# scroll-tech/zkevm-circuits

Hardware: AMD Instinct MI355X
Metric: SuperCircuit-shape proof-gen wall-clock (s) at k = 20 (lower is better)
Workload: dtype u32x8 limbs (254-bit modular integer, Montgomery)

## Files before the change

zkevm-circuits_amd/csrc/ntt.hip:

```cpp
#include "ctx.hpp"
#include "ff29.hip.hpp"

namespace zk {

constexpr int NTT_MAX_DIGIT = 10;
constexpr int NTT_TILE = 4096;
constexpr int NTT_THREADS = 1024;
constexpr int NTT_LDS_BYTES_PER_ELT = 36;

struct Tw29;

constexpr int NTT_BATCH = 16;
struct NttIo { const Fr* src[NTT_BATCH]; Fr* dst[NTT_BATCH]; };

struct NttPass {
    int log_np;
    int log_m;
    const Tw29* tw;
    const Fr* out_tw = nullptr;
};

struct NttDomain {
    uint32_t log_n = 0;
    int npass = 0;
    NttPass pass[3];
    int h = 0;
    Fr* d_lo = nullptr;
    Fr* d_hi = nullptr;
    Fr* d_tw[3] = {nullptr, nullptr, nullptr};
    Tw29* d_tw29[3] = {nullptr, nullptr, nullptr};
    Fr* d_out_tw[2] = {nullptr, nullptr};
    Fr final_mul;
    bool fin_folded = false;
    ~NttDomain() {
        if (d_lo) (void)hipFree(d_lo);
        if (d_hi) (void)hipFree(d_hi);
        for (auto p : d_tw) if (p) (void)hipFree(p);
        for (auto p : d_tw29) if (p) (void)hipFree((void*)p);
        for (auto p : d_out_tw) if (p) (void)hipFree(p);
    }
};

__device__ __forceinline__ uint32_t bitrev(uint32_t x, int bits) { return bits ? (__brev(x) >> (32 - bits)) : 0u; }

__host__ __device__ __forceinline__ Fr to_rprime(Fr x) {
#pragma unroll
    for (int i = 0; i < 5; ++i) x = dbl(x);
    return x;
}

struct Lds29 {
    uint32_t* p;
    int stride;
    __device__ __forceinline__ Fr29 load(int idx) const {
        Fr29 r;
#pragma unroll
        for (int k = 0; k < 9; ++k) r.l[k] = p[k * stride + idx];
        return r;
    }
    __device__ __forceinline__ void store(int idx, const Fr29& v) const {
#pragma unroll
        for (int k = 0; k < 9; ++k) p[k * stride + idx] = v.l[k];
    }
};

__global__ void k_powers(Fr base, Fr mul, Fr* out, uint32_t count, int rprime) {
    uint32_t j = blockIdx.x * blockDim.x + threadIdx.x;
    if (j >= count) return;
    Fr r = mul, b = base;
    uint32_t e = j;
    while (e) {
        if (e & 1) r = r * b;
        b = sqr(b);
        e >>= 1;
    }
    stg(out + j, rprime ? to_rprime(r) : r);
}

__device__ __forceinline__ Fr two_level(const Fr* __restrict__ lo, const Fr* __restrict__ hi, int h, uint32_t e) {
    return ldg(lo + (e & ((1u << h) - 1))) * ldg(hi + (e >> h));
}
__device__ __forceinline__ Fr29 two_level29(const Fr* __restrict__ lo, const Fr* __restrict__ hi, int h, uint32_t e) {
    return mul29(unpack29<Fr29P>(ldg(lo + (e & ((1u << h) - 1)))), unpack29<Fr29P>(ldg(hi + (e >> h))));
}

__global__ void k_build_out_twiddles(Fr* __restrict__ out_tw, const Fr* __restrict__ lo, const Fr* __restrict__ hi, int h, int log_np, int log_m, int tw_shift, uint64_t n,
                                     Fr fin, int apply_fin) {
    const uint64_t g = (uint64_t)blockIdx.x * blockDim.x + threadIdx.x;
    if (g >= n) return;
    const uint64_t m = 1ull << log_m;
    const uint32_t jpp = (uint32_t)(g & (m - 1)), d = (uint32_t)(g >> log_m) & ((1u << log_np) - 1);
    Fr29 v = two_level29(lo, hi, h, (jpp * d) << tw_shift);
    if (apply_fin) v = mul29(v, unpack29<Fr29P>(fin));
    stg(out_tw + g, pack29_lt2p(v));
}

__device__ __forceinline__ void bfly29(Fr29& u, Fr29& x, const Fr29& w) {
    const Fr29 v = mul29(x, w);
    Fr29 a0 = add29(u, v), a1 = sub29k<4>(u, v);
    normalize29(a0);
    normalize29(a1);
    u = a0;
    x = a1;
}
struct Tw29 { uint4 q[3]; };
__device__ __forceinline__ Fr29 tw29(const Tw29* __restrict__ tw, uint32_t idx) {
    const uint4 a = tw[idx].q[0], b = tw[idx].q[1], c = tw[idx].q[2];
    return Fr29{{a.x, a.y, a.z, a.w, b.x, b.y, b.z, b.w, c.x}};
}
__global__ void k_split_twiddles(const Fr* __restrict__ in, Tw29* __restrict__ out, uint32_t count) {
    const uint32_t i = blockIdx.x * blockDim.x + threadIdx.x;
    if (i >= count) return;
    const Fr29 v = unpack29<Fr29P>(ldg(in + i));
    out[i].q[0] = make_uint4(v.l[0], v.l[1], v.l[2], v.l[3]);
    out[i].q[1] = make_uint4(v.l[4], v.l[5], v.l[6], v.l[7]);
    out[i].q[2] = make_uint4(v.l[8], 0u, 0u, 0u);
}
__device__ __forceinline__ void bfly29_lazy(Fr29& u, Fr29& x, const Fr29& w) {
    const Fr29 v = mul29(x, w);
    const Fr29 a0 = add29(u, v), a1 = sub29k<2>(u, v);
    u = a0;
    x = a1;
}
template <int R>
__device__ __forceinline__ void dit_step(Fr29 (&e)[4], const Tw29* __restrict__ tw, int log_np, int s, int j) {
    const Fr29 w0 = tw29(tw, (uint32_t)j << (log_np - 1 - s));
    bfly29_lazy(e[0], e[1], w0);
    if (R == 2) {
        bfly29_lazy(e[2], e[3], w0);
        bfly29_lazy(e[0], e[2], tw29(tw, (uint32_t)j << (log_np - 2 - s)));
        bfly29_lazy(e[1], e[3], tw29(tw, (uint32_t)(j + (1 << s)) << (log_np - 2 - s)));
        normalize29(e[2]);
        normalize29(e[3]);
    }
    normalize29(e[0]);
    normalize29(e[1]);
}
__device__ __forceinline__ void bfly29_one(Fr29& u, Fr29& x) {
    Fr29 a0 = add29(u, x), a1 = sub29k<4>(u, x);
    normalize29(a0);
    normalize29(a1);
    u = a0;
    x = a1;
}
template <int R>
__device__ __forceinline__ void dit_first_step(Fr29 (&e)[4], const Tw29* __restrict__ tw, int log_np) {
    bfly29_one(e[0], e[1]);
    if (R == 2) {
        bfly29_one(e[2], e[3]);
        bfly29_one(e[0], e[2]);
        bfly29(e[1], e[3], tw29(tw, 1u << (log_np - 2)));
    }
}

__global__ void __launch_bounds__(NTT_THREADS)
k_ntt_pass(NttIo io, const Tw29* __restrict__ tw, const Fr* __restrict__ lo,
           const Fr* __restrict__ hi, int h, int log_np, int log_t, int log_m, int tw_shift, const Fr* __restrict__ pre,
           const Fr* __restrict__ out_tw, uint32_t ncols, int xcd_cols) {
    extern __shared__ __attribute__((aligned(16))) uint32_t smem[];
    uint32_t tile_id, col;
    if (xcd_cols) { const uint32_t slot = blockIdx.x >> 3; col = slot % ncols; tile_id = (slot / ncols) * 8u + (blockIdx.x & 7u); }
    else { col = blockIdx.x % ncols; tile_id = blockIdx.x / ncols; }
    const Fr* __restrict__ src = io.src[col];
    Fr* __restrict__ dst = io.dst[col];
    const int tile = 1 << (log_np + log_t);
    Lds29 L{smem, tile};
    const int T = 1 << log_t;
    const uint64_t m = 1ull << log_m;
    const uint32_t tiles_per_hi = (uint32_t)(m >> log_t);
    const uint32_t hi_idx = tile_id / tiles_per_hi, blk = tile_id % tiles_per_hi;
    const uint64_t base = ((uint64_t)hi_idx << (log_np + log_m)) + ((uint64_t)blk << log_t);

    for (int s = 0; s < log_np;) {
        const int r = ((log_np - s) & 1) ? 1 : 2;
        const bool first = s == 0, last = s + r == log_np;
        const int hgt = 1 << s, items = tile >> r;
        for (int it = threadIdx.x; it < items; it += blockDim.x) {
            const int c = it & (T - 1), b = it >> log_t;
            const int j = b & (hgt - 1);
            const int lo_d = ((b >> s) << (s + r)) | j;
            Fr29 e[4];
#pragma unroll
            for (int k = 0; k < 4; ++k) {
                if (k >= (1 << r)) break;
                const int dl = lo_d + k * hgt;
                if (first) {
                    const uint64_t gi = base + (uint64_t)bitrev(dl, log_np) * m + c;
                    e[k] = unpack29<Fr29P>(ldg(src + gi));
                    if (pre) e[k] = mul29(e[k], unpack29<Fr29P>(ldg(pre + gi)));
                } else {
                    e[k] = L.load((dl << log_t) | c);
                }
            }
            if (first) { if (r == 2) dit_first_step<2>(e, tw, log_np); else dit_first_step<1>(e, tw, log_np); }
            else if (r == 2) dit_step<2>(e, tw, log_np, s, j);
            else dit_step<1>(e, tw, log_np, s, j);
#pragma unroll
            for (int k = 0; k < 4; ++k) {
                if (k >= (1 << r)) break;
                const int dl = lo_d + k * hgt;
                if (last) {
                    const uint32_t jpp = (blk << log_t) + c;
                    const uint64_t go = base + (uint64_t)dl * m + c;
                    const Fr29 v = mul29(e[k], out_tw ? unpack29<Fr29P>(ldg(out_tw + go)) : two_level29(lo, hi, h, (jpp * (uint32_t)dl) << tw_shift));
                    stg(dst + go, pack29_raw(v));
                } else {
                    L.store((dl << log_t) | c, e[k]);
                }
            }
        }
        s += r;
        if (s < log_np) __syncthreads();
    }
}

static bool ntt_xcd_remap() { static const bool on = getenv("ZK_NTT_XCD") && atoi(getenv("ZK_NTT_XCD")) == 1; return on; }
__host__ __device__ __forceinline__ int ntt_row_pad(int log_np) { return log_np >= 8 ? 8 : 0; }
__global__ void __launch_bounds__(NTT_THREADS)
k_ntt_last(NttIo io, const Tw29* __restrict__ tw, int log_np, int log_t,
           int log_n1, int log_mid, Fr fin, const Fr* __restrict__ pre, int fin_folded, int xcd_remap) {
    extern __shared__ __attribute__((aligned(16))) uint32_t smem[];
    const Fr* __restrict__ src = io.src[blockIdx.y];
    Fr* __restrict__ dst = io.dst[blockIdx.y];
    const int tile = 1 << (log_np + log_t);
    const int T = 1 << log_t;
    const int row = (1 << log_np) + ntt_row_pad(log_np);
    Lds29 L{smem, T * row};
    uint32_t bx = blockIdx.x;
    if (xcd_remap) bx = (bx & 7u) * (gridDim.x >> 3) + (bx >> 3);
    const uint32_t mid = bx & ((1u << log_mid) - 1), blk = bx >> log_mid;
    const Fr29 fin29 = unpack29<Fr29P>(fin);

    for (int s = 0; s < log_np;) {
        const int r = ((log_np - s) & 1) ? 1 : 2;
        const bool first = s == 0, last = s + r == log_np;
        const int hgt = 1 << s, items = tile >> r;
        for (int it = threadIdx.x; it < items; it += blockDim.x) {
            int c, b;
            if (last) { c = it & (T - 1); b = it >> log_t; }
            else { b = it & ((1 << (log_np - r)) - 1); c = it >> (log_np - r); }
            const int j = b & (hgt - 1);
            const int lo_d = ((b >> s) << (s + r)) | j;
            const uint64_t i1 = ((uint64_t)blk << log_t) + c;
            Fr29 e[4];
#pragma unroll
            for (int k = 0; k < 4; ++k) {
                if (k >= (1 << r)) break;
                const int dl = lo_d + k * hgt;
                if (first) {
                    const uint64_t gi = (((i1 << log_mid) + mid) << log_np) + bitrev(dl, log_np);
                    e[k] = unpack29<Fr29P>(ldg(src + gi));
                    if (pre) e[k] = mul29(e[k], unpack29<Fr29P>(ldg(pre + gi)));
                } else {
                    e[k] = L.load(c * row + dl);
                }
            }
            if (first) { if (r == 2) dit_first_step<2>(e, tw, log_np); else dit_first_step<1>(e, tw, log_np); }
            else if (r == 2) dit_step<2>(e, tw, log_np, s, j);
            else dit_step<1>(e, tw, log_np, s, j);
#pragma unroll
            for (int k = 0; k < 4; ++k) {
                if (k >= (1 << r)) break;
                const int dl = lo_d + k * hgt;
                if (last) {
                    const uint64_t o = i1 + (((uint64_t)mid + ((uint64_t)dl << log_mid)) << log_n1);
                    stg(dst + o, fin_folded ? reduce_lazy29(e[k]) : pack29_lt2p(mul29(e[k], fin29)));
                } else {
                    L.store(c * row + dl, e[k]);
                }
            }
        }
        s += r;
        if (s < log_np) __syncthreads();
    }
}


template <int LOG_NP, int S, bool HAS_PRE>
__device__ __forceinline__ void ntt_pass_steps(const Lds29& L, const Fr* __restrict__ src, Fr* __restrict__ dst, const Tw29* __restrict__ tw,
                                               const Fr* __restrict__ pre, const Fr* __restrict__ out_tw, const int log_t, const uint64_t m, const uint64_t base) {
    constexpr int R = ((LOG_NP - S) & 1) ? 1 : 2, NE = 1 << R, hgt = 1 << S;
    constexpr bool FIRST = S == 0, LAST = S + R == LOG_NP;
    const int T = 1 << log_t, items = (1 << (LOG_NP + log_t)) >> R;
    for (int it = threadIdx.x; it < items; it += blockDim.x) {
        const int c = it & (T - 1), b = it >> log_t;
        const int j = b & (hgt - 1);
        const int lo_d = ((b >> S) << (S + R)) | j;
        Fr otw[NE];
        if (LAST) {
#pragma unroll
            for (int k = 0; k < NE; ++k) otw[k] = ldg(out_tw + base + (uint64_t)(lo_d + k * hgt) * m + c);
        }
        Fr29 e[4];
        if (FIRST) {
            Fr raw[NE], praw[NE];
#pragma unroll
            for (int k = 0; k < NE; ++k) {
                const uint64_t gi = base + (uint64_t)bitrev(lo_d + k * hgt, LOG_NP) * m + c;
                raw[k] = ldg(src + gi);
                if (HAS_PRE) praw[k] = ldg(pre + gi);
            }
#pragma unroll
            for (int k = 0; k < NE; ++k) {
                e[k] = unpack29<Fr29P>(raw[k]);
                if (HAS_PRE) e[k] = mul29(e[k], unpack29<Fr29P>(praw[k]));
            }
            dit_first_step<R>(e, tw, LOG_NP);
        } else {
#pragma unroll
            for (int k = 0; k < NE; ++k) e[k] = L.load(((lo_d + k * hgt) << log_t) | c);
            dit_step<R>(e, tw, LOG_NP, S, j);
        }
#pragma unroll
        for (int k = 0; k < NE; ++k) {
            const int dl = lo_d + k * hgt;
            if (LAST) stg(dst + base + (uint64_t)dl * m + c, pack29_raw(mul29(e[k], unpack29<Fr29P>(otw[k]))));
            else L.store((dl << log_t) | c, e[k]);
        }
    }
    if constexpr (!LAST) {
        __syncthreads();
        ntt_pass_steps<LOG_NP, S + R, HAS_PRE>(L, src, dst, tw, pre, out_tw, log_t, m, base);
    }
}
template <int LOG_NP, bool HAS_PRE>
__global__ void __launch_bounds__(NTT_THREADS)
k_ntt_pass_f(NttIo io, const Tw29* __restrict__ tw, int log_t, int log_m, const Fr* __restrict__ pre, const Fr* __restrict__ out_tw, uint32_t ncols, int xcd_cols, int log_grp) {
    extern __shared__ __attribute__((aligned(16))) uint32_t smem[];
    uint32_t tile_id, col;
    if (xcd_cols) {
        const uint32_t slot = blockIdx.x >> 3, sub = slot & ((1u << log_grp) - 1u), s2 = slot >> log_grp;
        col = s2 % ncols;
        tile_id = ((((s2 / ncols) << 3) + (blockIdx.x & 7u)) << log_grp) + sub;
    } else { col = blockIdx.x % ncols; tile_id = blockIdx.x / ncols; }
    Lds29 L{smem, 1 << (LOG_NP + log_t)};
    const uint64_t m = 1ull << log_m;
    const uint32_t tiles_per_hi = (uint32_t)(m >> log_t);
    const uint32_t hi_idx = tile_id / tiles_per_hi, blk = tile_id % tiles_per_hi;
    const uint64_t base = ((uint64_t)hi_idx << (LOG_NP + log_m)) + ((uint64_t)blk << log_t);
    ntt_pass_steps<LOG_NP, 0, HAS_PRE>(L, io.src[col], io.dst[col], tw, pre, out_tw, log_t, m, base);
}

template <int LOG_NP, int S>
__device__ __forceinline__ void ntt_last_steps(const Lds29& L, const Fr* __restrict__ src, Fr* __restrict__ dst, const Tw29* __restrict__ tw,
                                               const int log_t, const int row, const uint32_t blk, const uint32_t mid, const int log_mid, const int log_n1) {
    constexpr int R = ((LOG_NP - S) & 1) ? 1 : 2, NE = 1 << R, hgt = 1 << S;
    constexpr bool FIRST = S == 0, LAST = S + R == LOG_NP;
    const int T = 1 << log_t, items = (1 << (LOG_NP + log_t)) >> R;
    for (int it = threadIdx.x; it < items; it += blockDim.x) {
        int c, b;
        if (LAST) { c = it & (T - 1); b = it >> log_t; }
        else { b = it & ((1 << (LOG_NP - R)) - 1); c = it >> (LOG_NP - R); }
        const int j = b & (hgt - 1);
        const int lo_d = ((b >> S) << (S + R)) | j;
        const uint64_t i1 = ((uint64_t)blk << log_t) + c;
        Fr29 e[4];
        if (FIRST) {
            Fr raw[NE];
#pragma unroll
            for (int k = 0; k < NE; ++k) raw[k] = ldg(src + ((((i1 << log_mid) + mid) << LOG_NP) + bitrev(lo_d + k * hgt, LOG_NP)));
#pragma unroll
            for (int k = 0; k < NE; ++k) e[k] = unpack29<Fr29P>(raw[k]);
            dit_first_step<R>(e, tw, LOG_NP);
        } else {
#pragma unroll
            for (int k = 0; k < NE; ++k) e[k] = L.load(c * row + lo_d + k * hgt);
            dit_step<R>(e, tw, LOG_NP, S, j);
        }
#pragma unroll
        for (int k = 0; k < NE; ++k) {
            const int dl = lo_d + k * hgt;
            if (LAST) stg(dst + (i1 + (((uint64_t)mid + ((uint64_t)dl << log_mid)) << log_n1)), reduce_lazy29(e[k]));
            else L.store(c * row + dl, e[k]);
        }
    }
    if constexpr (!LAST) {
        __syncthreads();
        ntt_last_steps<LOG_NP, S + R>(L, src, dst, tw, log_t, row, blk, mid, log_mid, log_n1);
    }
}
template <int LOG_NP>
__global__ void __launch_bounds__(NTT_THREADS)
k_ntt_last_f(NttIo io, const Tw29* __restrict__ tw, int log_t, int log_n1, int log_mid, int xcd_remap) {
    extern __shared__ __attribute__((aligned(16))) uint32_t smem[];
    const int row = (1 << LOG_NP) + ntt_row_pad(LOG_NP);
    Lds29 L{smem, (1 << log_t) * row};
    uint32_t bx = blockIdx.x;
    if (xcd_remap) bx = (bx & 7u) * (gridDim.x >> 3) + (bx >> 3);
    const uint32_t mid = bx & ((1u << log_mid) - 1), blk = bx >> log_mid;
    ntt_last_steps<LOG_NP, 0>(L, io.src[blockIdx.y], io.dst[blockIdx.y], tw, log_t, row, blk, mid, log_mid, log_n1);
}

__global__ void k_scale(Fr* a, Fr s, uint64_t n) {
    uint64_t i = (uint64_t)blockIdx.x * blockDim.x + threadIdx.x;
    if (i < n) stg(a + i, ldg(a + i) * s);
}
int fr_scale_run(zk_ctx* ctx, Fr* d_a, const Fr& s, uint64_t n) {
    if (!n) return ZK_OK;
    hipLaunchKernelGGL(k_scale, dim3((unsigned)((n + 255) / 256)), dim3(256), 0, ctx->stream, d_a, s, n);
    ZK_CHECK_LAUNCH(ctx);
    return ZK_OK;
}

__global__ void k_distribute_powers(const Fr* src, Fr* dst, const Fr* __restrict__ lo, const Fr* __restrict__ hi, int h, uint64_t n) {
    uint64_t i = (uint64_t)blockIdx.x * blockDim.x + threadIdx.x;
    if (i >= n) return;
    stg(dst + i, ldg(src + i) * two_level(lo, hi, h, (uint32_t)i));
}

static int build_powers(zk_ctx* ctx, const Fr& base, const Fr& mul, Fr* d_out, uint32_t count, int rprime) {
    hipLaunchKernelGGL(k_powers, dim3((count + 255) / 256), dim3(256), 0, ctx->stream, base, mul, d_out, count, rprime);
    ZK_CHECK_LAUNCH(ctx);
    return ZK_OK;
}

static uint64_t domain_key(uint32_t log_n, const Fr& omega, const Fr* scale) {
    uint64_t hsh = 1469598103934665603ull;
    auto mix = [&](uint32_t v) { hsh = (hsh ^ v) * 1099511628211ull; };
    mix(log_n);
    for (int i = 0; i < 8; ++i) mix(omega.l[i]);
    if (scale) for (int i = 0; i < 8; ++i) mix(scale->l[i] ^ 0x9e3779b9u);
    return hsh;
}

static int get_domain(zk_ctx* ctx, uint32_t log_n, const Fr& omega, const Fr* scale, std::shared_ptr<NttDomain>* out) {
    const uint64_t key = domain_key(log_n, omega, scale);
    auto it = ctx->domains.find(key);
    if (it != ctx->domains.end()) { *out = it->second; return ZK_OK; }
    auto d = std::make_shared<NttDomain>();
    d->log_n = log_n;
    d->final_mul = to_rprime(scale ? *scale : Fr::one());
    const int P = log_n <= NTT_MAX_DIGIT ? 1 : (log_n <= 2 * NTT_MAX_DIGIT ? 2 : 3);
    d->npass = P;
    int rem = (int)log_n;
    for (int p = 0; p < P; ++p) {
        int b = (rem + (P - p) - 1) / (P - p);
        d->pass[p].log_np = b;
        rem -= b;
        d->pass[p].log_m = rem;
    }
    if (P > 1) {
        d->h = (int)(log_n + 1) / 2;
        const uint32_t nlo = 1u << d->h, nhi = 1u << (log_n - d->h);
        ZK_HIP(ctx, hipMalloc(&d->d_lo, sizeof(Fr) * nlo));
        ZK_HIP(ctx, hipMalloc(&d->d_hi, sizeof(Fr) * nhi));
        int rc = build_powers(ctx, omega, Fr::one(), d->d_lo, nlo, 1);
        if (rc) return rc;
        Fr step = omega;
        for (int i = 0; i < d->h; ++i) step = sqr(step);
        rc = build_powers(ctx, step, Fr::one(), d->d_hi, nhi, 1);
        if (rc) return rc;
    }
    for (int p = 0; p < P; ++p) {
        const int b = d->pass[p].log_np;
        const uint32_t cnt = b ? (1u << (b - 1)) : 1u;
        ZK_HIP(ctx, hipMalloc(&d->d_tw[p], sizeof(Fr) * cnt));
        Fr w = omega;
        for (uint32_t i = 0; i < log_n - (uint32_t)b; ++i) w = sqr(w);
        int rc = build_powers(ctx, w, Fr::one(), d->d_tw[p], cnt, 1);
        if (rc) return rc;
        ZK_HIP(ctx, hipMalloc((void**)&d->d_tw29[p], sizeof(Tw29) * cnt));
        hipLaunchKernelGGL(k_split_twiddles, dim3((cnt + 255) / 256), dim3(256), 0, ctx->stream, (const Fr*)d->d_tw[p], d->d_tw29[p], cnt);
        ZK_CHECK_LAUNCH(ctx);
        d->pass[p].tw = d->d_tw29[p];
    }
    if (P > 1 && log_n <= 24) {
        const uint64_t n = 1ull << log_n;
        for (int p = 0; p + 1 < P; ++p) {
            if (hipMalloc(&d->d_out_tw[p], sizeof(Fr) * n) != hipSuccess) { (void)hipGetLastError(); d->d_out_tw[p] = nullptr; break; }
            const NttPass& ps = d->pass[p];
            hipLaunchKernelGGL(k_build_out_twiddles, dim3((unsigned)((n + 255) / 256)), dim3(256), 0, ctx->stream, d->d_out_tw[p], (const Fr*)d->d_lo, (const Fr*)d->d_hi, d->h,
                               ps.log_np, ps.log_m, (int)log_n - ps.log_np - ps.log_m, n, d->final_mul, p == P - 2 ? 1 : 0);
            ZK_CHECK_LAUNCH(ctx);
            d->pass[p].out_tw = d->d_out_tw[p];
            if (p == P - 2) d->fin_folded = true;
        }
    }
    if (ctx->domains.size() > 64) ctx->domains.clear();
    ctx->domains[key] = d;
    *out = d;
    return ZK_OK;
}

static int set_lds_attr(zk_ctx* ctx) {
    if (ctx->ntt_attr_set) return ZK_OK;
    ZK_HIP(ctx, hipFuncSetAttribute((const void*)k_ntt_pass, hipFuncAttributeMaxDynamicSharedMemorySize, NTT_TILE * NTT_LDS_BYTES_PER_ELT));
    ZK_HIP(ctx, hipFuncSetAttribute((const void*)k_ntt_last, hipFuncAttributeMaxDynamicSharedMemorySize, (NTT_TILE + 128) * NTT_LDS_BYTES_PER_ELT));
    ctx->ntt_attr_set = true;
    return ZK_OK;
}


template <int LOG_NP, bool HAS_PRE>
static bool launch_pass_f(zk_ctx* ctx, unsigned grid, unsigned threads, size_t lds, const NttIo& io, const Tw29* tw, int log_t, int log_m, const Fr* pre, const Fr* out_tw, uint32_t ncols, int xcd_cols, int log_grp) {
    const uint32_t bit = 1u << (2 * (LOG_NP - 7) + (HAS_PRE ? 1 : 0));
    if (!(ctx->ntt_fixed_attr & bit)) {
        if (hipFuncSetAttribute((const void*)k_ntt_pass_f<LOG_NP, HAS_PRE>, hipFuncAttributeMaxDynamicSharedMemorySize, NTT_TILE * NTT_LDS_BYTES_PER_ELT) != hipSuccess) { (void)hipGetLastError(); return false; }
        ctx->ntt_fixed_attr |= bit;
    }
    hipLaunchKernelGGL((k_ntt_pass_f<LOG_NP, HAS_PRE>), dim3(grid), dim3(threads), lds, ctx->stream, io, tw, log_t, log_m, pre, out_tw, ncols, xcd_cols, log_grp);
    return true;
}
static bool ntt_fixed_on() { const char* e = getenv("ZK_NTT_FIXED"); return !(e && atoi(e) == 0); }
static bool launch_pass_fixed(zk_ctx* ctx, int log_np, unsigned grid, unsigned threads, size_t lds, const NttIo& io, const Tw29* tw, int log_t, int log_m, const Fr* pre, const Fr* out_tw, uint32_t ncols, int xcd_cols, int log_grp) {
    if (!ntt_fixed_on() || !out_tw) return false;
#define ZK_PASS_CASE(N) case N: return pre ? launch_pass_f<N, true>(ctx, grid, threads, lds, io, tw, log_t, log_m, pre, out_tw, ncols, xcd_cols, log_grp) \
                                           : launch_pass_f<N, false>(ctx, grid, threads, lds, io, tw, log_t, log_m, pre, out_tw, ncols, xcd_cols, log_grp);
    switch (log_np) { ZK_PASS_CASE(7) ZK_PASS_CASE(8) ZK_PASS_CASE(9) ZK_PASS_CASE(10) ZK_PASS_CASE(11) default: return false; }
#undef ZK_PASS_CASE
}
template <int LOG_NP>
static bool launch_last_f(zk_ctx* ctx, dim3 grid, unsigned threads, size_t lds, const NttIo& io, const Tw29* tw, int log_t, int log_n1, int log_mid, int xcd_remap) {
    const uint32_t bit = 1u << (24 + LOG_NP - 7);
    if (!(ctx->ntt_fixed_attr & bit)) {
        if (hipFuncSetAttribute((const void*)k_ntt_last_f<LOG_NP>, hipFuncAttributeMaxDynamicSharedMemorySize, (NTT_TILE + 128) * NTT_LDS_BYTES_PER_ELT) != hipSuccess) { (void)hipGetLastError(); return false; }
        ctx->ntt_fixed_attr |= bit;
    }
    hipLaunchKernelGGL((k_ntt_last_f<LOG_NP>), grid, dim3(threads), lds, ctx->stream, io, tw, log_t, log_n1, log_mid, xcd_remap);
    return true;
}
static bool launch_last_fixed(zk_ctx* ctx, int log_np, dim3 grid, unsigned threads, size_t lds, const NttIo& io, const Tw29* tw, int log_t, int log_n1, int log_mid, int xcd_remap) {
    if (!ntt_fixed_on()) return false;
#define ZK_LAST_CASE(N) case N: return launch_last_f<N>(ctx, grid, threads, lds, io, tw, log_t, log_n1, log_mid, xcd_remap);
    switch (log_np) { ZK_LAST_CASE(7) ZK_LAST_CASE(8) ZK_LAST_CASE(9) ZK_LAST_CASE(10) ZK_LAST_CASE(11) default: return false; }
#undef ZK_LAST_CASE
}

static int pick_threads(int tile) { return tile >= 4096 ? 1024 : (tile >= 1024 ? 512 : (tile >= 256 ? 128 : 64)); }

int ntt_run_many(zk_ctx* ctx, Fr* const* d_datas, const Fr* const* d_srcs, size_t count, uint32_t log_n, const Fr& omega, const Fr* scale, const Fr* coset_pre, const Fr* coset_post, bool fuse_pre);
int ntt_run(zk_ctx* ctx, Fr* d_data, uint32_t log_n, const Fr& omega, const Fr* scale, const Fr* coset_pre, const Fr* coset_post, const Fr* d_src, bool fuse_pre) {
    return ntt_run_many(ctx, &d_data, d_src ? &d_src : nullptr, 1, log_n, omega, scale, coset_pre, coset_post, fuse_pre);
}
int ntt_run_many(zk_ctx* ctx, Fr* const* d_datas, const Fr* const* d_srcs, size_t count, uint32_t log_n, const Fr& omega, const Fr* scale, const Fr* coset_pre, const Fr* coset_post, bool fuse_pre) {
    if (count == 0) return ZK_OK;
    if (count > 1 && (log_n == 0 || coset_post)) {
        for (size_t i = 0; i < count; ++i) {
            const Fr* one_src = d_srcs ? d_srcs[i] : nullptr;
            int r = ntt_run_many(ctx, d_datas + i, one_src ? &one_src : nullptr, 1, log_n, omega, scale, coset_pre, coset_post, fuse_pre);
            if (r) return r;
        }
        return ZK_OK;
    }
    Fr* d_data = d_datas[0];
    const Fr* d_src = d_srcs ? d_srcs[0] : nullptr;
    if (log_n == 0) {
        if (d_src && d_src != d_data) ZK_HIP(ctx, hipMemcpyAsync(d_data, d_src, sizeof(Fr), hipMemcpyDeviceToDevice, ctx->stream));
        if (scale) {
            hipLaunchKernelGGL(k_scale, dim3(1), dim3(64), 0, ctx->stream, d_data, *scale, (uint64_t)1);
            ZK_CHECK_LAUNCH(ctx);
        }
        return ZK_OK;
    }
    int rc = set_lds_attr(ctx);
    if (rc) return rc;
    const uint64_t n = 1ull << log_n;

    auto run_distribute = [&](const Fr& g, const Fr* from) -> int {
        const int h = (int)(log_n + 1) / 2;
        const uint32_t nlo = 1u << h, nhi = 1u << (log_n - h);
        const uint64_t key = domain_key(log_n, g, nullptr) ^ 0xC05E7ull;
        Fr* tab = nullptr;
        auto it = ctx->pow_tables.find(key);
        if (it != ctx->pow_tables.end()) {
            tab = (Fr*)it->second;
        } else {
            if (hipMalloc(&tab, sizeof(Fr) * ((size_t)nlo + nhi)) != hipSuccess) return ctx->fail(ZK_ERR_OOM, "coset table allocation failed");
            int r = build_powers(ctx, g, Fr::one(), tab, nlo, 0);
            if (r) return r;
            Fr step = g;
            for (int i = 0; i < h; ++i) step = sqr(step);
            r = build_powers(ctx, step, Fr::one(), tab + nlo, nhi, 0);
            if (r) return r;
            ctx->pow_tables[key] = tab;
        }
        hipLaunchKernelGGL(k_distribute_powers, dim3((unsigned)((n + 255) / 256)), dim3(256), 0, ctx->stream, from, d_data, tab, tab + nlo, h, n);
        ZK_CHECK_LAUNCH(ctx);
        return ZK_OK;
    };
    const Fr* cur = d_src ? d_src : d_data;
    const Fr* pre_table = nullptr;
    if (coset_pre && fuse_pre) {
        const uint64_t key = domain_key(log_n, *coset_pre, nullptr) ^ 0xF0117ABull;
        auto it = ctx->pow_tables.find(key);
        if (it != ctx->pow_tables.end()) {
            pre_table = (const Fr*)it->second;
        } else {
            Fr* tab = nullptr;
            if (hipMalloc(&tab, sizeof(Fr) * n) != hipSuccess) { (void)hipGetLastError(); tab = nullptr; }
            if (tab) {
                int r = build_powers(ctx, *coset_pre, Fr::one(), tab, (uint32_t)n, 1);
                if (r) return r;
                ctx->pow_tables[key] = tab;
                pre_table = tab;
            }
        }
    }
    if (coset_pre && !pre_table) {
        if (count > 1) {
            for (size_t i = 0; i < count; ++i) {
                const Fr* one_src = d_srcs ? d_srcs[i] : nullptr;
                int r = ntt_run_many(ctx, d_datas + i, one_src ? &one_src : nullptr, 1, log_n, omega, scale, coset_pre, coset_post, fuse_pre);
                if (r) return r;
            }
            return ZK_OK;
        }
        rc = run_distribute(*coset_pre, cur); if (rc) return rc; cur = d_data;
    }

    std::shared_ptr<NttDomain> dom;
    rc = get_domain(ctx, log_n, omega, scale, &dom);
    if (rc) return rc;
    const int P = dom->npass;
    size_t per_launch = 1;
    if (count > 1) {
        const uint64_t tiles = std::max<uint64_t>(1, n >> 12);
        per_launch = (size_t)std::min<uint64_t>(NTT_BATCH, std::max<uint64_t>(1, 4096 / tiles));
        if (const char* e = getenv("ZK_NTT_BATCH")) { const int v = atoi(e); if (v >= 1 && v <= NTT_BATCH) per_launch = (size_t)v; }
    }
    Fr* scratch = nullptr;
    if (P > 1) {
        const int slot = ctx->stream_aux && ctx->stream == ctx->stream_aux ? SC_NTT_AUX : SC_NTT;
        for (;;) {
            scratch = (Fr*)ctx->get_scratch(slot, sizeof(Fr) * n * per_launch);
            if (scratch || per_launch == 1) break;
            (void)hipGetLastError();
            per_launch = (per_launch + 1) / 2;
        }
        if (!scratch) return ZK_ERR_OOM;
    }
    for (size_t first = 0; first < count; first += per_launch) {
        const size_t nb = std::min(per_launch, count - first);
        NttIo io_in{}, io_mid{}, io_last{};
        for (size_t j = 0; j < nb; ++j) {
            Fr* dd = d_datas[first + j];
            const Fr* ss = (count == 1) ? cur : (d_srcs && d_srcs[first + j] ? d_srcs[first + j] : dd);
            io_in.src[j] = ss;
            io_in.dst[j] = dd;
        }
        NttIo cur_io = io_in;
        for (int p = 0; p + 1 < P; ++p) {
            const NttPass& ps = dom->pass[p];
            int log_tile_pass = P == 3 ? 11 : 12;
            if (const char* e = getenv("ZK_NTT_PASS_LOGTILE")) { const int v = atoi(e); if (v >= 10 && v <= 12) log_tile_pass = v; }
            int log_t = log_tile_pass - ps.log_np;
            if (log_t < 0) log_t = 0;
            if (log_t > ps.log_m) log_t = ps.log_m;
            const int tile = 1 << (ps.log_np + log_t);
            NttIo io{};
            for (size_t j = 0; j < nb; ++j) {
                io.src[j] = cur_io.src[j];
                io.dst[j] = (p == P - 2) ? scratch + j * n : d_datas[first + j];
            }
            const unsigned blocks = (unsigned)(n >> (ps.log_np + log_t));
            const int tw_shift = (int)log_n - ps.log_np - ps.log_m;
            ZkProfScope pscope(ctx, "ntt_pass");
            pscope.bytes = (uint64_t)nb * n * 64 / (uint64_t)P;
            static const bool xcd_off = getenv("ZK_NTT_XCD_COLS") && atoi(getenv("ZK_NTT_XCD_COLS")) == 0;
            const int xcd_cols = (nb > 1 && blocks % 8 == 0 && !xcd_off) ? 1 : 0;
            const int log_grp = log_t < 2 ? 2 - log_t : 0;
            const int xcd_fixed = (!xcd_off && blocks % (8u << log_grp) == 0 && (nb > 1 || log_grp > 0)) ? 1 : 0;
            if (!launch_pass_fixed(ctx, ps.log_np, blocks * (unsigned)nb, (unsigned)std::max(64, std::min(1024, tile >> 2)) , (size_t)tile * NTT_LDS_BYTES_PER_ELT, io, ps.tw, log_t, ps.log_m,
                                   p == 0 ? pre_table : (const Fr*)nullptr, ps.out_tw, (uint32_t)nb, xcd_fixed, xcd_fixed ? log_grp : 0))
                hipLaunchKernelGGL(k_ntt_pass, dim3(blocks * (unsigned)nb), dim3(pick_threads(tile)), (size_t)tile * NTT_LDS_BYTES_PER_ELT, ctx->stream, io, ps.tw,
                                   dom->d_lo, dom->d_hi, dom->h, ps.log_np, log_t, ps.log_m, tw_shift, p == 0 ? pre_table : (const Fr*)nullptr, ps.out_tw,
                                   (uint32_t)nb, xcd_cols);
            ZK_CHECK_LAUNCH(ctx);
            for (size_t j = 0; j < nb; ++j) cur_io.src[j] = io.dst[j];
        }
        {
            const NttPass& ps = dom->pass[P - 1];
            const int log_n1 = P == 1 ? 0 : dom->pass[0].log_np;
            const int log_mid = P == 3 ? dom->pass[1].log_np : 0;
            int log_tile_last = 11;
            if (const char* e = getenv("ZK_NTT_LAST_LOGTILE")) { const int v = atoi(e); if (v >= 10 && v <= 12) log_tile_last = v; }
            int log_t = log_tile_last - ps.log_np;
            if (log_t < 0) log_t = 0;
            if (log_t > log_n1) log_t = log_n1;
            const int tile = 1 << (ps.log_np + log_t);
            const unsigned blocks = (unsigned)(n >> (ps.log_np + log_t));
            NttIo io{};
            for (size_t j = 0; j < nb; ++j) { io.src[j] = cur_io.src[j]; io.dst[j] = d_datas[first + j]; }
            ZkProfScope pscope(ctx, "ntt_last");
            pscope.bytes = (uint64_t)nb * n * 64 / (uint64_t)P;
            const int xcd_last = (log_mid == 0 && blocks % 8 == 0 && blocks >= 16 && ntt_xcd_remap()) ? 1 : 0;
            const size_t lds_last = (size_t)(tile + (ntt_row_pad(ps.log_np) << log_t)) * NTT_LDS_BYTES_PER_ELT;
            if (!(P > 1 && dom->fin_folded && launch_last_fixed(ctx, ps.log_np, dim3(blocks, (unsigned)nb), (unsigned)std::max(64, std::min(1024, tile >> 2)), lds_last, io, ps.tw, log_t, log_n1, log_mid, xcd_last)))
                hipLaunchKernelGGL(k_ntt_last, dim3(blocks, (unsigned)nb), dim3(pick_threads(tile)), lds_last, ctx->stream, io, ps.tw,
                                   ps.log_np, log_t, log_n1, log_mid, dom->final_mul, P == 1 ? pre_table : (const Fr*)nullptr, dom->fin_folded ? 1 : 0, xcd_last);
            ZK_CHECK_LAUNCH(ctx);
        }
    }
    if (coset_post) { rc = run_distribute(*coset_post, d_data); if (rc) return rc; }
    return ZK_OK;
}

template <int W>
__global__ void __launch_bounds__(256) k_ntt_cross(const Fr* __restrict__ recv, Fr* __restrict__ out, size_t cols, const Fr* __restrict__ tw , Fr scale, int scaled) {
    const size_t c = (size_t)blockIdx.x * blockDim.x + threadIdx.x;
    if (c >= cols) return;
    constexpr int LOGW = W == 2 ? 1 : W == 4 ? 2 : W == 8 ? 3 : 4;
    Fr a[W];
#pragma unroll
    for (int i = 0; i < W; ++i) {
        int rev = 0;
#pragma unroll
        for (int b = 0; b < LOGW; ++b) rev |= ((i >> b) & 1) << (LOGW - 1 - b);
        a[rev] = ldg(recv + (size_t)i * cols + c);
    }
#pragma unroll
    for (int st = 1; st <= LOGW; ++st) {
#pragma unroll
        for (int h = 0; h < W / 2; ++h) {
            const int half = 1 << (st - 1), t = h & (half - 1), lo = ((h >> (st - 1)) << st) + t, hi = lo + half;
            const Fr u = a[lo];
            const Fr v = t == 0 ? a[hi] : a[hi] * tw[t << (LOGW - st)];
            a[lo] = u + v;
            a[hi] = u - v;
        }
    }
#pragma unroll
    for (int j = 0; j < W; ++j) stg(out + (size_t)j * cols + c, scaled ? a[j] * scale : a[j]);
}

}

using namespace zk;
extern "C" int zk_ntt_sharded(zk_ctx* ctx, void* d_local, uint32_t log_n, int inverse, uint32_t rank, uint32_t world, zk_alltoall_fn exchange, void* user) {
    if (!ctx) return ZK_ERR_INVALID_ARG;
    ZK_REQUIRE(ctx, d_local, "null pointer");
    ZK_REQUIRE(ctx, exchange || world == 1 || (comm_ready(ctx) && ctx->comm_world == world && ctx->comm_rank == rank), "no all-to-all callback and no matching communicator (zk_comm_init)");
    ZK_REQUIRE(ctx, world >= 1 && world <= 16 && (world & (world - 1)) == 0 && rank < world, "world must be a power of two <= 16, rank < world");
    ZK_REQUIRE(ctx, log_n <= 28, "log_n exceeds the two-adicity of Fr (28)");
    uint32_t log_w = 0;
    while ((1u << log_w) < world) ++log_w;
    ZK_REQUIRE(ctx, log_n >= 2 * log_w, "need n >= world^2");
    if (world == 1) return zk_ntt(ctx, d_local, log_n, inverse);
    const uint32_t log_m = log_n - log_w;
    const size_t m = (size_t)1 << log_m, cols = m >> log_w;
    Fr w_n = fr_root_of_unity(log_n), w_m = fr_root_of_unity(log_m), w_w = fr_root_of_unity(log_w);
    if (inverse) { w_n = fr_inv_host(w_n); w_m = fr_inv_host(w_m); w_w = fr_inv_host(w_w); }
    const Fr g = fr_pow(w_n, rank);
    int rc = ntt_run(ctx, (Fr*)d_local, log_m, w_m, nullptr, nullptr, rank ? &g : nullptr);
    if (rc) return rc;
    Fr* recv = (Fr*)ctx->pool_get(m * sizeof(Fr));
    Fr* d_tw = (Fr*)ctx->pool_get(16 * sizeof(Fr));
    if (!recv || !d_tw) { ctx->pool_put(recv, m * sizeof(Fr)); ctx->pool_put(d_tw, 16 * sizeof(Fr)); return ctx->fail(ZK_ERR_OOM, "sharded NTT: exchange buffer of %zu bytes", m * sizeof(Fr)); }
    auto done = [&](int code) { ctx->pool_put(recv, m * sizeof(Fr)); ctx->pool_put(d_tw, 16 * sizeof(Fr)); return code; };
    hipError_t e = hipSuccess;
    if (exchange) {
        e = hipStreamSynchronize(ctx->stream);
        if (e != hipSuccess) return done(ctx->fail(ZK_ERR_HIP, "sharded NTT: %s", hipGetErrorString(e)));
        if (exchange(user, d_local, cols * sizeof(Fr), recv) != 0) return done(ctx->fail(ZK_ERR_INVALID_ARG, "sharded NTT: the all-to-all callback failed"));
    } else {
        rc = comm_alltoall_dev(ctx, d_local, cols * sizeof(Fr), recv);
        if (rc) return done(rc);
    }
    Fr tw[8];
    tw[0] = Fr::one();
    for (uint32_t t = 1; t < (world > 1 ? world / 2 : 1); ++t) tw[t] = tw[t - 1] * w_w;
    e = hipMemcpyAsync(d_tw, tw, sizeof(Fr) * (world / 2 ? world / 2 : 1), hipMemcpyHostToDevice, ctx->stream);
    if (e != hipSuccess) return done(ctx->fail(ZK_ERR_HIP, "sharded NTT: %s", hipGetErrorString(e)));
    const Fr ninv = inverse ? fr_inv_host(fr_from_u64(1ull << log_n)) : Fr::one();
    const dim3 grid((unsigned)((cols + 255) / 256)), block(256);
    switch (world) {
        case 2: hipLaunchKernelGGL(k_ntt_cross<2>, grid, block, 0, ctx->stream, (const Fr*)recv, (Fr*)d_local, cols, (const Fr*)d_tw, ninv, inverse); break;
        case 4: hipLaunchKernelGGL(k_ntt_cross<4>, grid, block, 0, ctx->stream, (const Fr*)recv, (Fr*)d_local, cols, (const Fr*)d_tw, ninv, inverse); break;
        case 8: hipLaunchKernelGGL(k_ntt_cross<8>, grid, block, 0, ctx->stream, (const Fr*)recv, (Fr*)d_local, cols, (const Fr*)d_tw, ninv, inverse); break;
        default: hipLaunchKernelGGL(k_ntt_cross<16>, grid, block, 0, ctx->stream, (const Fr*)recv, (Fr*)d_local, cols, (const Fr*)d_tw, ninv, inverse); break;
    }
    e = hipGetLastError();
    if (e != hipSuccess) return done(ctx->fail(ZK_ERR_HIP, "sharded NTT: %s", hipGetErrorString(e)));
    e = hipStreamSynchronize(ctx->stream);
    if (e != hipSuccess) return done(ctx->fail(ZK_ERR_HIP, "sharded NTT: %s", hipGetErrorString(e)));
    return done(ZK_OK);
}
```

Before: 1.869.

## Run inner NTT radix-4 steps per-wavefront with swizzled LDS layout

Remaps the LDS layout of the fixed-size NTT pass and last kernels so that every 256-element group holds whole sub-butterflies for one wavefront, with an XOR swizzle to spread accesses across LDS banks. Middle radix-4 steps whose span fits within that group run as wave-local loops, and consecutive such steps are separated by a wavefront fence plus wave barrier in place of a block-wide __syncthreads. The aim is fewer workgroup barriers and fewer LDS bank conflicts. In exchange the indexing is more complex, and tiles smaller than 256 elements fall back to the generic path.

After: 1.868 (median of 2 runs). About the same (-0.1%).

```diff
diff --git a/zkevm-circuits_amd/csrc/ntt.hip b/zkevm-circuits_amd/csrc/ntt.hip
--- a/zkevm-circuits_amd/csrc/ntt.hip
+++ b/zkevm-circuits_amd/csrc/ntt.hip
@@ -276,50 +276,89 @@
 }
 
 
+constexpr int NTT_WAVE_LOG_ELTS = 8;
+__host__ __device__ constexpr int ntt_wave_log_digits(int log_np) { return log_np < NTT_WAVE_LOG_ELTS ? log_np : NTT_WAVE_LOG_ELTS; }
+__device__ __forceinline__ int ntt_swz(int x) { return x ^ ((x >> 3) & 0xC) ^ ((x >> 2) & 0x10); }
+__device__ __forceinline__ void ntt_wave_sync() {
+    __builtin_amdgcn_fence(__ATOMIC_RELEASE, "wavefront");
+    __builtin_amdgcn_wave_barrier();
+    __builtin_amdgcn_fence(__ATOMIC_ACQUIRE, "wavefront");
+}
+template <int LOG_NP, int S>
+struct NttStep {
+    static constexpr int R = ((LOG_NP - S) & 1) ? 1 : 2, NE = 1 << R, hgt = 1 << S;
+    static constexpr bool FIRST = S == 0, LAST = S + R == LOG_NP;
+    static constexpr bool WAVE = !FIRST && !LAST && R == 2 && S + R <= ntt_wave_log_digits(LOG_NP);
+};
+template <int LOG_NP>
+__device__ __forceinline__ int ntt_pass_idx(const int d, const int c, const int log_t) {
+    constexpr int B = ntt_wave_log_digits(LOG_NP), LOG_CW = NTT_WAVE_LOG_ELTS - B;
+    const int q = ((d >> B) << (log_t - LOG_CW)) | (c >> LOG_CW);
+    const int x = ((c & ((1 << LOG_CW) - 1)) << B) | (d & ((1 << B) - 1));
+    return (q << NTT_WAVE_LOG_ELTS) | (ntt_swz(x) ^ ((q & 3) * 9));
+}
 template <int LOG_NP, int S, bool HAS_PRE>
 __device__ __forceinline__ void ntt_pass_steps(const Lds29& L, const Fr* __restrict__ src, Fr* __restrict__ dst, const Tw29* __restrict__ tw,
                                                const Fr* __restrict__ pre, const Fr* __restrict__ out_tw, const int log_t, const uint64_t m, const uint64_t base) {
-    constexpr int R = ((LOG_NP - S) & 1) ? 1 : 2, NE = 1 << R, hgt = 1 << S;
-    constexpr bool FIRST = S == 0, LAST = S + R == LOG_NP;
-    const int T = 1 << log_t, items = (1 << (LOG_NP + log_t)) >> R;
-    for (int it = threadIdx.x; it < items; it += blockDim.x) {
-        const int c = it & (T - 1), b = it >> log_t;
-        const int j = b & (hgt - 1);
-        const int lo_d = ((b >> S) << (S + R)) | j;
-        Fr otw[NE];
-        if (LAST) {
-#pragma unroll
-            for (int k = 0; k < NE; ++k) otw[k] = ldg(out_tw + base + (uint64_t)(lo_d + k * hgt) * m + c);
-        }
-        Fr29 e[4];
-        if (FIRST) {
-            Fr raw[NE], praw[NE];
+    using St = NttStep<LOG_NP, S>;
+    constexpr int R = St::R, NE = St::NE, hgt = St::hgt;
+    constexpr bool FIRST = St::FIRST, LAST = St::LAST;
+    if constexpr (St::WAVE) {
+        constexpr int B = ntt_wave_log_digits(LOG_NP), LOG_CW = NTT_WAVE_LOG_ELTS - B;
+        const int lane = threadIdx.x & 63, nblocks = 1 << (LOG_NP + log_t - NTT_WAVE_LOG_ELTS);
+        const int bl = lane & ((1 << (B - 2)) - 1), j = bl & (hgt - 1);
+        const int x0 = ((lane >> (B - 2)) << B) | ((bl >> S) << (S + 2)) | j;
+        for (int q = threadIdx.x >> 6; q < nblocks; q += blockDim.x >> 6) {
+            const int at = q << NTT_WAVE_LOG_ELTS, cx = (q & 3) * 9;
+            Fr29 e[4];
+#pragma unroll
+            for (int k = 0; k < 4; ++k) e[k] = L.load(at | (ntt_swz(x0 + k * hgt) ^ cx));
+            dit_step<2>(e, tw, LOG_NP, S, j);
+#pragma unroll
+            for (int k = 0; k < 4; ++k) L.store(at | (ntt_swz(x0 + k * hgt) ^ cx), e[k]);
+        }
+    } else {
+        const int T = 1 << log_t, items = (1 << (LOG_NP + log_t)) >> R;
+        for (int it = threadIdx.x; it < items; it += blockDim.x) {
+            const int c = it & (T - 1), b = it >> log_t;
+            const int j = b & (hgt - 1);
+            const int lo_d = ((b >> S) << (S + R)) | j;
+            Fr otw[NE];
+            if (LAST) {
+#pragma unroll
+                for (int k = 0; k < NE; ++k) otw[k] = ldg(out_tw + base + (uint64_t)(lo_d + k * hgt) * m + c);
+            }
+            Fr29 e[4];
+            if (FIRST) {
+                Fr raw[NE], praw[NE];
+#pragma unroll
+                for (int k = 0; k < NE; ++k) {
+                    const uint64_t gi = base + (uint64_t)bitrev(lo_d + k * hgt, LOG_NP) * m + c;
+                    raw[k] = ldg(src + gi);
+                    if (HAS_PRE) praw[k] = ldg(pre + gi);
+                }
+#pragma unroll
+                for (int k = 0; k < NE; ++k) {
+                    e[k] = unpack29<Fr29P>(raw[k]);
+                    if (HAS_PRE) e[k] = mul29(e[k], unpack29<Fr29P>(praw[k]));
+                }
+                dit_first_step<R>(e, tw, LOG_NP);
+            } else {
+#pragma unroll
+                for (int k = 0; k < NE; ++k) e[k] = L.load(ntt_pass_idx<LOG_NP>(lo_d + k * hgt, c, log_t));
+                dit_step<R>(e, tw, LOG_NP, S, j);
+            }
 #pragma unroll
             for (int k = 0; k < NE; ++k) {
-                const uint64_t gi = base + (uint64_t)bitrev(lo_d + k * hgt, LOG_NP) * m + c;
-                raw[k] = ldg(src + gi);
-                if (HAS_PRE) praw[k] = ldg(pre + gi);
-            }
-#pragma unroll
-            for (int k = 0; k < NE; ++k) {
-                e[k] = unpack29<Fr29P>(raw[k]);
-                if (HAS_PRE) e[k] = mul29(e[k], unpack29<Fr29P>(praw[k]));
-            }
-            dit_first_step<R>(e, tw, LOG_NP);
-        } else {
-#pragma unroll
-            for (int k = 0; k < NE; ++k) e[k] = L.load(((lo_d + k * hgt) << log_t) | c);
-            dit_step<R>(e, tw, LOG_NP, S, j);
-        }
-#pragma unroll
-        for (int k = 0; k < NE; ++k) {
-            const int dl = lo_d + k * hgt;
-            if (LAST) stg(dst + base + (uint64_t)dl * m + c, pack29_raw(mul29(e[k], unpack29<Fr29P>(otw[k]))));
-            else L.store((dl << log_t) | c, e[k]);
+                const int dl = lo_d + k * hgt;
+                if (LAST) stg(dst + base + (uint64_t)dl * m + c, pack29_raw(mul29(e[k], unpack29<Fr29P>(otw[k]))));
+                else L.store(ntt_pass_idx<LOG_NP>(dl, c, log_t), e[k]);
+            }
         }
     }
     if constexpr (!LAST) {
-        __syncthreads();
+        if constexpr (St::WAVE && NttStep<LOG_NP, S + R>::WAVE) ntt_wave_sync();
+        else __syncthreads();
         ntt_pass_steps<LOG_NP, S + R, HAS_PRE>(L, src, dst, tw, pre, out_tw, log_t, m, base);
     }
 }
@@ -341,41 +380,65 @@
     ntt_pass_steps<LOG_NP, 0, HAS_PRE>(L, io.src[col], io.dst[col], tw, pre, out_tw, log_t, m, base);
 }
 
+template <int LOG_NP>
+__device__ __forceinline__ int ntt_last_idx(const int c, const int d, const int row) {
+    if constexpr (LOG_NP >= NTT_WAVE_LOG_ELTS) return c * row + (d & ~255) + ntt_swz(d & 255);
+    else { const int f = (c << LOG_NP) | d; return (f & ~255) | ntt_swz(f & 255); }
+}
 template <int LOG_NP, int S>
 __device__ __forceinline__ void ntt_last_steps(const Lds29& L, const Fr* __restrict__ src, Fr* __restrict__ dst, const Tw29* __restrict__ tw,
                                                const int log_t, const int row, const uint32_t blk, const uint32_t mid, const int log_mid, const int log_n1) {
-    constexpr int R = ((LOG_NP - S) & 1) ? 1 : 2, NE = 1 << R, hgt = 1 << S;
-    constexpr bool FIRST = S == 0, LAST = S + R == LOG_NP;
-    const int T = 1 << log_t, items = (1 << (LOG_NP + log_t)) >> R;
-    for (int it = threadIdx.x; it < items; it += blockDim.x) {
-        int c, b;
-        if (LAST) { c = it & (T - 1); b = it >> log_t; }
-        else { b = it & ((1 << (LOG_NP - R)) - 1); c = it >> (LOG_NP - R); }
-        const int j = b & (hgt - 1);
-        const int lo_d = ((b >> S) << (S + R)) | j;
-        const uint64_t i1 = ((uint64_t)blk << log_t) + c;
-        Fr29 e[4];
-        if (FIRST) {
-            Fr raw[NE];
-#pragma unroll
-            for (int k = 0; k < NE; ++k) raw[k] = ldg(src + ((((i1 << log_mid) + mid) << LOG_NP) + bitrev(lo_d + k * hgt, LOG_NP)));
-#pragma unroll
-            for (int k = 0; k < NE; ++k) e[k] = unpack29<Fr29P>(raw[k]);
-            dit_first_step<R>(e, tw, LOG_NP);
-        } else {
-#pragma unroll
-            for (int k = 0; k < NE; ++k) e[k] = L.load(c * row + lo_d + k * hgt);
-            dit_step<R>(e, tw, LOG_NP, S, j);
-        }
-#pragma unroll
-        for (int k = 0; k < NE; ++k) {
-            const int dl = lo_d + k * hgt;
-            if (LAST) stg(dst + (i1 + (((uint64_t)mid + ((uint64_t)dl << log_mid)) << log_n1)), reduce_lazy29(e[k]));
-            else L.store(c * row + dl, e[k]);
+    using St = NttStep<LOG_NP, S>;
+    constexpr int R = St::R, NE = St::NE, hgt = St::hgt;
+    constexpr bool FIRST = St::FIRST, LAST = St::LAST;
+    if constexpr (St::WAVE) {
+        constexpr int B = ntt_wave_log_digits(LOG_NP);
+        const int lane = threadIdx.x & 63, nblocks = 1 << (LOG_NP + log_t - NTT_WAVE_LOG_ELTS);
+        const int bl = lane & ((1 << (B - 2)) - 1), j = bl & (hgt - 1);
+        const int x0 = ((lane >> (B - 2)) << B) | ((bl >> S) << (S + 2)) | j;
+        for (int q = threadIdx.x >> 6; q < nblocks; q += blockDim.x >> 6) {
+            const int f = q << NTT_WAVE_LOG_ELTS;
+            const int at = LOG_NP >= NTT_WAVE_LOG_ELTS ? (f >> LOG_NP) * row + (f & ((1 << LOG_NP) - 1)) : f;
+            Fr29 e[4];
+#pragma unroll
+            for (int k = 0; k < 4; ++k) e[k] = L.load(at + ntt_swz(x0 + k * hgt));
+            dit_step<2>(e, tw, LOG_NP, S, j);
+#pragma unroll
+            for (int k = 0; k < 4; ++k) L.store(at + ntt_swz(x0 + k * hgt), e[k]);
+        }
+    } else {
+        const int T = 1 << log_t, items = (1 << (LOG_NP + log_t)) >> R;
+        for (int it = threadIdx.x; it < items; it += blockDim.x) {
+            int c, b;
+            if (LAST) { c = it & (T - 1); b = it >> log_t; }
+            else { b = it & ((1 << (LOG_NP - R)) - 1); c = it >> (LOG_NP - R); }
+            const int j = b & (hgt - 1);
+            const int lo_d = ((b >> S) << (S + R)) | j;
+            const uint64_t i1 = ((uint64_t)blk << log_t) + c;
+            Fr29 e[4];
+            if (FIRST) {
+                Fr raw[NE];
+#pragma unroll
+                for (int k = 0; k < NE; ++k) raw[k] = ldg(src + ((((i1 << log_mid) + mid) << LOG_NP) + bitrev(lo_d + k * hgt, LOG_NP)));
+#pragma unroll
+                for (int k = 0; k < NE; ++k) e[k] = unpack29<Fr29P>(raw[k]);
+                dit_first_step<R>(e, tw, LOG_NP);
+            } else {
+#pragma unroll
+                for (int k = 0; k < NE; ++k) e[k] = L.load(ntt_last_idx<LOG_NP>(c, lo_d + k * hgt, row));
+                dit_step<R>(e, tw, LOG_NP, S, j);
+            }
+#pragma unroll
+            for (int k = 0; k < NE; ++k) {
+                const int dl = lo_d + k * hgt;
+                if (LAST) stg(dst + (i1 + (((uint64_t)mid + ((uint64_t)dl << log_mid)) << log_n1)), reduce_lazy29(e[k]));
+                else L.store(ntt_last_idx<LOG_NP>(c, dl, row), e[k]);
+            }
         }
     }
     if constexpr (!LAST) {
-        __syncthreads();
+        if constexpr (St::WAVE && NttStep<LOG_NP, S + R>::WAVE) ntt_wave_sync();
+        else __syncthreads();
         ntt_last_steps<LOG_NP, S + R>(L, src, dst, tw, log_t, row, blk, mid, log_mid, log_n1);
     }
 }
@@ -503,7 +566,7 @@
 }
 static bool ntt_fixed_on() { const char* e = getenv("ZK_NTT_FIXED"); return !(e && atoi(e) == 0); }
 static bool launch_pass_fixed(zk_ctx* ctx, int log_np, unsigned grid, unsigned threads, size_t lds, const NttIo& io, const Tw29* tw, int log_t, int log_m, const Fr* pre, const Fr* out_tw, uint32_t ncols, int xcd_cols, int log_grp) {
-    if (!ntt_fixed_on() || !out_tw) return false;
+    if (!ntt_fixed_on() || !out_tw || log_np + log_t < NTT_WAVE_LOG_ELTS) return false;
 #define ZK_PASS_CASE(N) case N: return pre ? launch_pass_f<N, true>(ctx, grid, threads, lds, io, tw, log_t, log_m, pre, out_tw, ncols, xcd_cols, log_grp) \
                                            : launch_pass_f<N, false>(ctx, grid, threads, lds, io, tw, log_t, log_m, pre, out_tw, ncols, xcd_cols, log_grp);
     switch (log_np) { ZK_PASS_CASE(7) ZK_PASS_CASE(8) ZK_PASS_CASE(9) ZK_PASS_CASE(10) ZK_PASS_CASE(11) default: return false; }
@@ -520,7 +583,7 @@
     return true;
 }
 static bool launch_last_fixed(zk_ctx* ctx, int log_np, dim3 grid, unsigned threads, size_t lds, const NttIo& io, const Tw29* tw, int log_t, int log_n1, int log_mid, int xcd_remap) {
-    if (!ntt_fixed_on()) return false;
+    if (!ntt_fixed_on() || log_np + log_t < NTT_WAVE_LOG_ELTS) return false;
 #define ZK_LAST_CASE(N) case N: return launch_last_f<N>(ctx, grid, threads, lds, io, tw, log_t, log_n1, log_mid, xcd_remap);
     switch (log_np) { ZK_LAST_CASE(7) ZK_LAST_CASE(8) ZK_LAST_CASE(9) ZK_LAST_CASE(10) ZK_LAST_CASE(11) default: return false; }
 #undef ZK_LAST_CASE
```
